# NVIDIA-Merlin/NVTabular

Measured on AMD Instinct MI355X. Metric: rows/sec + GB/s (Criteo Categorify+FillMissing+Normalize fit+transform, HBM-resident), higher is better.
Workload: dtype int32 keys -> int64 labels; fp64 moments/normalize; 1 GPU; synthetic Criteo-day0: 26 int32 categorical (Criteo-1TB cardinalities, Zipf) + 13 int32 continuous, nulls as Arrow bitmaps; Categorify + FillMissing + Normalize, fit + transform; rows_per_gpu=45000000, algorithmic_bytes_per_row=624, tie_break=value (count desc, value asc), artifacts=deferred (no parquet I/O inside the timed region)

## Files before the change

### nvtabular_amd/csrc/nvt_sort.hip

```cpp
#include <type_traits>

#include <cstdlib>
#include <vector>

#include "nvt_common.hpp"
#include "nvt_internal.hpp"
#include "nvt_prof.hpp"
#include "nvt_range.hpp"
#include "nvt_image.hpp"
#include "nvt_scan.hpp"

extern "C" int nvt_vocab_sort_tmp_bytes(int key_bytes, uint64_t n, uint64_t *bytes);

namespace nvt {

template <typename K>
__device__ __forceinline__ unsigned sort_digit(K key, int64_t cnt, int pass) {
  constexpr int KB = (int)sizeof(K);
  if (pass < KB) {
    using U = typename std::make_unsigned<K>::type;
    U u = (U)key ^ ((U)1 << (8 * KB - 1));
    return (unsigned)((u >> (8 * pass)) & 0xFF);
  }
  uint64_t inv = ~(uint64_t)cnt;
  return (unsigned)((inv >> (8 * (pass - KB))) & 0xFF);
}

constexpr int kSmallMax = 8192;
constexpr int kSmallBS = 1024;

template <typename K>
__device__ __forceinline__ bool vocab_before(int64_t ca, K ka, int64_t cb, K kb) {
  return ca > cb || (ca == cb && ka < kb);
}

template <typename K>
__global__ __launch_bounds__(kSmallBS) void sort_small_kernel(K *keys, int64_t *counts, unsigned n) {
  __shared__ K sk[kSmallMax];
  __shared__ int64_t sc[kSmallMax];
  unsigned m = 1;
  while (m < n) m <<= 1;
  for (unsigned i = threadIdx.x; i < m; i += kSmallBS) {
    if (i < n) {
      sk[i] = keys[i];
      sc[i] = counts[i];
    } else {
      sk[i] = std::numeric_limits<K>::max();
      sc[i] = INT64_MIN;
    }
  }
  __syncthreads();
  for (unsigned size = 2; size <= m; size <<= 1) {
    for (unsigned stride = size >> 1; stride > 0; stride >>= 1) {
      for (unsigned t = threadIdx.x; t < m / 2; t += kSmallBS) {
        unsigned lo = 2 * t - (t & (stride - 1));
        unsigned hi = lo + stride;
        bool up = (lo & size) == 0;
        K ka = sk[lo], kb = sk[hi];
        int64_t ca = sc[lo], cb = sc[hi];
        bool swap = up ? vocab_before<K>(cb, kb, ca, ka) : vocab_before<K>(ca, ka, cb, kb);
        if (swap) {
          sk[lo] = kb;
          sk[hi] = ka;
          sc[lo] = cb;
          sc[hi] = ca;
        }
      }
      __syncthreads();
    }
  }
  for (unsigned i = threadIdx.x; i < n; i += kSmallBS) {
    keys[i] = sk[i];
    counts[i] = sc[i];
  }
}

constexpr int kRows = 8;
constexpr int kTileSort = kBlock * kRows;

template <typename K>
__global__ __launch_bounds__(kBlock) void sort_pass_hist_kernel(const K *__restrict__ keys,
                                                                const int64_t *__restrict__ cnts,
                                                                uint64_t n,
                                                                unsigned long long *pass_hist) {
// ... 564 lines not shown
}

uint64_t sort_words_tmp_bytes(uint64_t n) { return os_tmp_bytes(n); }

static int sort_words_impl(uint64_t *data, const void *keys, int key_dtype, int64_t key_bias,
                           const uint8_t *fold, int rb, uint64_t n, int bit_lo, int bit_hi, void *tmp,
                           uint64_t **result, hipStream_t stream) {
  NVT_CHECK_ARG(n < (1ull << 30), "at most 2^30-1 words");
  const int npass = (bit_hi - bit_lo + 7) / 8;
  NVT_CHECK_ARG(npass >= 1 && npass <= kOsMaxPass, "bit range too wide");
  const uint64_t ntiles = (n + kS2Tile - 1) / kS2Tile;
  char *p = reinterpret_cast<char *>(tmp);
  uint64_t *bufs[2];
  bufs[0] = reinterpret_cast<uint64_t *>(p);
  p += n * 8;
  bufs[1] = reinterpret_cast<uint64_t *>(p);
  p += n * 8;
  unsigned *block_hist = reinterpret_cast<unsigned *>(p);
  p += (uint64_t)kOsHistBlocks * kOsMaxPass * 256 * 4;
  unsigned *base = reinterpret_cast<unsigned *>(p);
  p += kOsMaxPass * 256 * 4;
  unsigned *status = reinterpret_cast<unsigned *>(p);
  const uint64_t status_words = (uint64_t)npass * ntiles * 256;
  unsigned *tickets = status + status_words;
  NVT_CHECK_HIP(hipMemsetAsync(status, 0, (status_words + kOsMaxPass) * 4, stream));
  const unsigned hb = (unsigned)(ntiles < (uint64_t)kOsHistBlocks ? ntiles : kOsHistBlocks);
  const PackedKeyWord<int32_t> s32{reinterpret_cast<const int32_t *>(keys), fold, key_bias, rb};
  const PackedKeyWord<int64_t> s64{reinterpret_cast<const int64_t *>(keys), fold, key_bias, rb};
  if (!keys)
    os_hist_words_kernel<<<hb, kS2BS, 0, stream>>>(data, n, bit_lo, npass, block_hist);
  else if (key_dtype == NVT_I32)
    os_hist_pack_kernel<int32_t><<<hb, kS2BS, 0, stream>>>(s32, n, bit_lo, npass, block_hist);
  else
    os_hist_pack_kernel<int64_t><<<hb, kS2BS, 0, stream>>>(s64, n, bit_lo, npass, block_hist);
  NVT_CHECK_LAUNCH();
  os_base_kernel<<<npass, 256, 0, stream>>>(block_hist, (int)hb, base);
  NVT_CHECK_LAUNCH();
  const uint64_t *src = data;
  int flip = 0;
  for (int pass = 0; pass < npass; ++pass) {
    uint64_t *dst = bufs[flip];
    unsigned *st = status + (uint64_t)pass * ntiles * 256;
    if (pass == 0 && keys && key_dtype == NVT_I32)
      os_scatter_pack_kernel<int32_t><<<(unsigned)ntiles, kS2BS, 0, stream>>>(
          s32, n, bit_lo, base, st, tickets, dst);
    else if (pass == 0 && keys)
      os_scatter_pack_kernel<int64_t><<<(unsigned)ntiles, kS2BS, 0, stream>>>(
          s64, n, bit_lo, base, st, tickets, dst);
    else
      os_scatter_kernel<false, false><<<(unsigned)ntiles, kS2BS, 0, stream>>>(
          src, nullptr, nullptr, n, bit_lo + 8 * pass, base + pass * 256, st, tickets + pass, dst,
          nullptr, nullptr);
    NVT_CHECK_LAUNCH();
    src = dst;
    flip ^= 1;
  }
  *result = const_cast<uint64_t *>(src);
  return NVT_OK;
}

int sort_words_bits(uint64_t *data, uint64_t n, int bit_lo, int bit_hi, void *tmp, uint64_t **result,
                    hipStream_t stream) {
  *result = data;
  if (n <= 1 || bit_hi <= bit_lo) return NVT_OK;
  return sort_words_impl(data, nullptr, 0, 0, nullptr, 0, n, bit_lo, bit_hi, tmp, result, stream);
}

int sort_packed_keys(const void *keys, int key_dtype, int64_t key_bias, const uint8_t *fold, int rb,
                     uint64_t n, void *tmp, uint64_t **result, hipStream_t stream) {
  NVT_CHECK_ARG(keys && n >= 1 && rb >= 24 && rb <= 32, "keys / rows / row bits");
  return sort_words_impl(nullptr, keys, key_dtype, key_bias, fold, rb, n, rb, 64, tmp, result, stream);
}

constexpr int kSmallPackedMax = 16384;
struct SmallCol {
  int32_t *keys;
  int64_t *counts;
  unsigned n;
};
constexpr int kSmallBatch = 64;
struct SmallBatch {
  SmallCol c[kSmallBatch];
};
__global__ __launch_bounds__(kSmallBS) void sort_small_packed_many_kernel(SmallBatch b) {
  __shared__ uint64_t sv[kSmallPackedMax];
  const SmallCol col = b.c[blockIdx.x];
  const unsigned n = col.n;
  unsigned m = 1;
  while (m < n) m <<= 1;
  for (unsigned i = threadIdx.x; i < m; i += kSmallBS)
    sv[i] = i < n ? comp_make(col.keys[i], col.counts[i]) : ~0ull;
  __syncthreads();
  for (unsigned size = 2; size <= m; size <<= 1) {
    for (unsigned stride = size >> 1; stride > 0; stride >>= 1) {
      for (unsigned t = threadIdx.x; t < m / 2; t += kSmallBS) {
        const unsigned lo = 2 * t - (t & (stride - 1));
        const unsigned hi = lo + stride;
        const bool up = (lo & size) == 0;
        const uint64_t a = sv[lo], c = sv[hi];
        if (up ? (c < a) : (a < c)) {
          sv[lo] = c;
          sv[hi] = a;
        }
      }
      __syncthreads();
    }
  }
  for (unsigned i = threadIdx.x; i < n; i += kSmallBS) {
    const uint64_t v = sv[i];
    col.keys[i] = comp_key(v);
    col.counts[i] = comp_cnt(v);
  }
}

inline uint64_t sort2_tmp_bytes(uint64_t n) {
  const uint64_t ntiles = (n + kS2Tile - 1) / kS2Tile, hist_len = 256 * ntiles;
  return 2 * n * 8 + pad16(hist_len * 4) + scan_chunks(hist_len) * 8 + 64;
}

inline int vocab_sort_packed(int32_t *keys, int64_t *counts, uint64_t n, int64_t max_count,
                             void *tmp, hipStream_t stream) {
  const uint64_t ntiles = (n + kS2Tile - 1) / kS2Tile, hist_len = 256 * ntiles;
  char *p = reinterpret_cast<char *>(tmp);
  uint64_t *bufs[2];
  bufs[0] = reinterpret_cast<uint64_t *>(p);
  p += n * 8;
  bufs[1] = reinterpret_cast<uint64_t *>(p);
  p += n * 8;
  unsigned *tile_hist = reinterpret_cast<unsigned *>(p);
  p += pad16(hist_len * 4);
  unsigned long long *chunk_tot = reinterpret_cast<unsigned long long *>(p);
  int count_bytes = 0;
  for (uint64_t m = (uint64_t)max_count; m; m >>= 8) ++count_bytes;
  const int npass = 4 + count_bytes;
  const uint64_t *src = nullptr;
  int flip = 0;
  for (int pass = 0; pass < npass; ++pass) {
    const int shift = 8 * pass;
    const bool first = pass == 0, last = pass == npass - 1;
    if (first)
      sort2_hist_kernel<true><<<(unsigned)ntiles, kS2BS, 0, stream>>>(nullptr, keys, counts, n,
                                                                       shift, tile_hist, ntiles);
    else
      sort2_hist_kernel<false><<<(unsigned)ntiles, kS2BS, 0, stream>>>(src, nullptr, nullptr, n,
                                                                        shift, tile_hist, ntiles);
    NVT_CHECK_LAUNCH();
    const unsigned long long *cbase = nullptr;
    {
      int rc = exclusive_scan_u32_deferred(tile_hist, hist_len, chunk_tot, &cbase, stream);
      if (rc) return rc;
    }
    uint64_t *dst = bufs[flip];
    if (first)
      sort2_scatter_kernel<true, false><<<(unsigned)ntiles, kS2BS, 0, stream>>>(
          nullptr, keys, counts, n, shift, tile_hist, cbase, ntiles, dst, nullptr, nullptr);
    else if (last)
      sort2_scatter_kernel<false, true><<<(unsigned)ntiles, kS2BS, 0, stream>>>(
          src, nullptr, nullptr, n, shift, tile_hist, cbase, ntiles, nullptr, keys, counts);
    else
      sort2_scatter_kernel<false, false><<<(unsigned)ntiles, kS2BS, 0, stream>>>(
          src, nullptr, nullptr, n, shift, tile_hist, cbase, ntiles, dst, nullptr, nullptr);
    NVT_CHECK_LAUNCH();
    src = dst;
    flip ^= 1;
  }
  return NVT_OK;
}

template <typename K>
int vocab_sort(K *keys, int64_t *counts, uint64_t n, int64_t max_count, void *tmp,
               hipStream_t stream) {
  constexpr int NP = (int)sizeof(K) + 8;
  if (n <= 1) return NVT_OK;
  NVT_CHECK_ARG(n < (1ull << 32), "at most 2^32-1 vocabulary entries");
  if (n <= kSmallMax) {
    sort_small_kernel<K><<<1, kSmallBS, 0, stream>>>(keys, counts, (unsigned)n);
    NVT_CHECK_LAUNCH();
    return NVT_OK;
  }
  if constexpr (sizeof(K) == 4) {
    if (max_count > 0 && max_count < (1ll << 32) && n < (1ull << 30) && !ab_env("NVT_SORT_LEGACY"))
      return vocab_sort_onesweep(keys, counts, n, max_count, tmp, stream);
    if (max_count > 0 && max_count < (1ll << 32) && n < (1ull << 31))
      return vocab_sort_packed(keys, counts, n, max_count, tmp, stream);
  }
  const uint64_t ntiles = (n + kTileSort - 1) / kTileSort;
  char *p = reinterpret_cast<char *>(tmp);
  int64_t *counts2 = reinterpret_cast<int64_t *>(p);
  p += n * sizeof(int64_t);
  K *keys2 = reinterpret_cast<K *>(p);
  p += pad16(n * sizeof(K));
  unsigned *tile_hist = reinterpret_cast<unsigned *>(p);
  const uint64_t hist_len = 256 * ntiles;
  p += pad16(hist_len * sizeof(unsigned));
  const uint64_t nchunks = (hist_len + kScanChunk - 1) / kScanChunk;
  unsigned long long *chunk_tot = reinterpret_cast<unsigned long long *>(p);
  p += nchunks * sizeof(unsigned long long);
  unsigned long long *pass_hist = reinterpret_cast<unsigned long long *>(p);

  bool run_pass[NP];
  if (max_count > 0) {
    constexpr int KB = (int)sizeof(K);
    int count_bytes = 0;
    for (uint64_t m = (uint64_t)max_count; m; m >>= 8) ++count_bytes;
    for (int p = 0; p < NP; ++p) run_pass[p] = p < KB || (p - KB) < count_bytes;
  } else {
    NVT_CHECK_HIP(hipMemsetAsync(pass_hist, 0, NP * 256 * sizeof(unsigned long long), stream));
    sort_pass_hist_kernel<K><<<stream_grid(n, kBlock * 8, 4), kBlock, 0, stream>>>(keys, counts, n,
                                                                                     pass_hist);
    NVT_CHECK_LAUNCH();
    unsigned long long host_hist[NP * 256];
    NVT_CHECK_HIP(hipMemcpyAsync(host_hist, pass_hist, sizeof(host_hist), hipMemcpyDeviceToHost,
                                 stream));
    NVT_CHECK_HIP(hipStreamSynchronize(stream));
    for (int p = 0; p < NP; ++p) {
      run_pass[p] = true;
      for (int d = 0; d < 256; ++d)
        if (host_hist[p * 256 + d] == n) run_pass[p] = false;
    }
  }

  K *src_k = keys, *dst_k = keys2;
  int64_t *src_c = counts, *dst_c = counts2;
  for (int pass = 0; pass < NP; ++pass) {
    if (!run_pass[pass]) continue;
    sort_tile_hist_kernel<K><<<(unsigned)ntiles, kBlock, 0, stream>>>(src_k, src_c, n, pass,
                                                                      tile_hist, ntiles);
    NVT_CHECK_LAUNCH();
    {
      int rc = exclusive_scan_u32(tile_hist, hist_len, chunk_tot, stream);
      if (rc) return rc;
    }
    sort_scatter_kernel<K><<<(unsigned)ntiles, kBlock, 0, stream>>>(src_k, src_c, n, pass,
                                                                    tile_hist, ntiles, dst_k, dst_c);
    NVT_CHECK_LAUNCH();
    K *tk = src_k;
    src_k = dst_k;
    dst_k = tk;
    int64_t *tc = src_c;
    src_c = dst_c;
    dst_c = tc;
  }
  if (src_k != keys) {
    NVT_CHECK_HIP(hipMemcpyAsync(keys, src_k, n * sizeof(K), hipMemcpyDeviceToDevice, stream));
    NVT_CHECK_HIP(
        hipMemcpyAsync(counts, src_c, n * sizeof(int64_t), hipMemcpyDeviceToDevice, stream));
  }
  return NVT_OK;
}

int vocab_sort_any(int key_bytes, void *keys, int64_t *counts, uint64_t n, int64_t max_count,
                   void *tmp, hipStream_t s) {
  NVT_PROF("vocab_sort", 0, s);
  if (key_bytes == 4) return vocab_sort<int32_t>((int32_t *)keys, counts, n, max_count, tmp, s);
  return vocab_sort<int64_t>((int64_t *)keys, counts, n, max_count, tmp, s);
}

bool vocab_sort_small_eligible(int key_bytes, uint64_t n, int64_t max_count) {
  return key_bytes == 4 && n >= 2 && n <= (uint64_t)kSmallPackedMax && max_count > 0 &&
         max_count < (1ll << 32);
}

int vocab_sort_small_batch(const SmallSortDesc *cols, int ncols, hipStream_t s) {
  for (int c0 = 0; c0 < ncols; c0 += kSmallBatch) {
    const int nc = ncols - c0 < kSmallBatch ? ncols - c0 : kSmallBatch;
    SmallBatch b;
    memset(&b, 0, sizeof(b));
    for (int i = 0; i < nc; ++i) {
      b.c[i].keys = cols[c0 + i].keys;
      b.c[i].counts = cols[c0 + i].counts;
      b.c[i].n = cols[c0 + i].n;
    }
    NVT_PROF("vocab_sort_small", 0, s);
    sort_small_packed_many_kernel<<<nc, kSmallBS, 0, s>>>(b);
    NVT_CHECK_LAUNCH();
  }
  return NVT_OK;
}

__device__ __forceinline__ unsigned cls_digit(uint64_t comp) {
  const uint32_t cnt = ~(uint32_t)(comp >> 32);
  return 255u - (cnt < 255u ? cnt : 255u);
}

__device__ __forceinline__ void cls_scatter_body(
    const int32_t *__restrict__ keys, const int64_t *__restrict__ cnts, uint64_t n,
    const unsigned *__restrict__ cls_hist, unsigned *status, unsigned *ticket, int32_t *out_keys,
    int64_t *out_cnts, unsigned long long *table, uint64_t mask, int64_t first_label,
    int64_t *sentinel_label, int32_t *label_of, int32_t *big_src = nullptr) {
  constexpr int NW = kS2BS / kWave;
  __shared__ unsigned wcnt[NW][256];
  __shared__ unsigned goff[256];
  __shared__ unsigned wtot[NW], btot[NW];
  __shared__ unsigned s_tile;
  __shared__ uint64_t stage[kS2Tile];
  const unsigned w = threadIdx.x / kWave, l = lane_id();
  if (threadIdx.x == 0) s_tile = atomicAdd(ticket, 1u);
#pragma unroll
  for (int q = 0; q < NW; ++q) wcnt[q][threadIdx.x] = 0;
  unsigned cbase;
  {
    const unsigned v = cls_hist[255 - threadIdx.x];
    unsigned inc = v;
#pragma unroll
    for (int off = 1; off < 64; off <<= 1) {
      unsigned o = __shfl_up(inc, off, 64);
      if (l >= (unsigned)off) inc += o;
    }
    if (l == 63) btot[w] = inc;
    __syncthreads();
    unsigned wb = 0;
    for (unsigned q = 0; q < w; ++q) wb += btot[q];
    cbase = wb + inc - v;
  }
  const unsigned tile = s_tile;
  uint64_t c[kS2Rows];
  unsigned short local[kS2Rows];
#pragma unroll
  for (int r = 0; r < kS2Rows; ++r) {
    const uint64_t i = s2_elem(tile, w, r, l);
    c[r] = ~0ull;
    if (i < n) c[r] = comp_make(keys[i], cnts[i]);
  }
  const uint64_t tile_base = (uint64_t)tile * kS2Tile;
#pragma unroll
  for (int r = 0; r < kS2Rows; ++r) {
    const bool act = s2_elem(tile, w, r, l) < n;
    const unsigned d = cls_digit(c[r]);
    const unsigned long long peers = match_digit(d, act);
    const unsigned rank = __popcll(peers & ((1ull << l) - 1ull));
    const unsigned before = act ? wcnt[w][d] : 0;
    __builtin_amdgcn_wave_barrier();
    if (act && rank == 0) wcnt[w][d] = before + (unsigned)__popcll(peers);
    __builtin_amdgcn_wave_barrier();
    local[r] = (unsigned short)(before + rank);
  }
  __syncthreads();
  {
    const unsigned d = threadIdx.x;
    unsigned t[NW], tot = 0;
#pragma unroll
    for (int q = 0; q < NW; ++q) {
      t[q] = wcnt[q][d];
      tot += t[q];
    }
    unsigned *my = status + (uint64_t)tile * 256 + d;
    __hip_atomic_store(my, (tile == 0 ? kOsPrefix : kOsAgg) | tot, __ATOMIC_RELAXED,
                       __HIP_MEMORY_SCOPE_AGENT);
    unsigned inc = tot;
#pragma unroll
    for (int off = 1; off < 64; off <<= 1) {
      unsigned o = __shfl_up(inc, off, 64);
      if (l >= (unsigned)off) inc += o;
    }
    if (l == 63) wtot[w] = inc;
    __syncthreads();
    unsigned wbase = 0;
    for (unsigned q = 0; q < w; ++q) wbase += wtot[q];
    const unsigned dstart = wbase + inc - tot;
    unsigned run = dstart;
#pragma unroll
    for (int q = 0; q < NW; ++q) {
      wcnt[q][d] = run;
      run += t[q];
    }
    unsigned excl = 0;
    if (tile > 0) {
      unsigned tb = tile - 1;
      while (true) {
        const unsigned v = __hip_atomic_load(status + (uint64_t)tb * 256 + d, __ATOMIC_RELAXED,
                                             __HIP_MEMORY_SCOPE_AGENT);
        const unsigned f = v >> 30;
        if (f == 0) {
          __builtin_amdgcn_s_sleep(1);
          continue;
        }
        excl += v & kOsMask;
        if (f == 2) break;
        --tb;
      }
      __hip_atomic_store(my, kOsPrefix | (excl + tot), __ATOMIC_RELAXED, __HIP_MEMORY_SCOPE_AGENT);
    }
    goff[d] = cbase + excl - dstart;
  }
  __syncthreads();
#pragma unroll
  for (int r = 0; r < kS2Rows; ++r) {
    const uint64_t i = s2_elem(tile, w, r, l);
    if (i < n) {
      const unsigned d = cls_digit(c[r]);
      const unsigned sidx = wcnt[w][d] + local[r];
      stage[sidx] = c[r];
      if (label_of != nullptr) label_of[i] = d != 0 ? (int32_t)(first_label + goff[d] + sidx) : -1;
      if (big_src != nullptr && d == 0) big_src[goff[0] + sidx] = (int32_t)i;
    }
  }
  __syncthreads();
  const unsigned tile_n = (unsigned)(n - tile_base < (uint64_t)kS2Tile ? n - tile_base : kS2Tile);
#pragma unroll 4
  for (int j = 0; j < kS2Rows; ++j) {
    const unsigned idx = j * kS2BS + threadIdx.x;
    if (idx < tile_n) {
      const uint64_t v = stage[idx];
      const unsigned d = cls_digit(v);
      if (big_src != nullptr && d != 0) continue;
      const unsigned dst = goff[d] + idx;
      const int32_t key = comp_key(v);
      out_keys[dst] = key;
      out_cnts[dst] = comp_cnt(v);
      if (key == INT32_MIN && d != 0 && sentinel_label != nullptr) {
        *sentinel_label = first_label + (int64_t)dst;
      } else if (table != nullptr && d != 0) {
        const int64_t label = first_label + (int64_t)dst;
        {
          const unsigned long long want = ((unsigned long long)(uint32_t)label << 32) | (uint32_t)key;
          uint64_t slot = (uint64_t)slot_hash(key) & mask;
          while (atomicCAS(&table[slot], kEncEmptySlot, want) != kEncEmptySlot) slot = (slot + 1) & mask;
        }
      }
    }
  }
}

__global__ __launch_bounds__(kS2BS) void cls_scatter_kernel(
    const int32_t *__restrict__ keys, const int64_t *__restrict__ cnts, uint64_t n,
    const unsigned *__restrict__ cls_hist, unsigned *status, unsigned *ticket, int32_t *out_keys,
    int64_t *out_cnts, unsigned long long *table, uint64_t mask, int64_t first_label,
    int64_t *sentinel_label, int32_t *label_of) {
  cls_scatter_body(keys, cnts, n, cls_hist, status, ticket, out_keys, out_cnts, table, mask,
                   first_label, sentinel_label, label_of);
}

constexpr int kOrdBatch = 16;
struct OrdJob {
  const int32_t *keys;
  const int64_t *cnts;
  const unsigned *cls_hist;
  unsigned *status, *ticket;
  int32_t *out_keys;
  int64_t *out_cnts;
  int32_t *label_of;
  unsigned long long *table;
  int64_t *sentinel_label;
  int32_t *aux;
  unsigned long long *fb_status;
  unsigned long long n, capacity, nslots, flat_slots, first_label, status_words, fb_words;
};
struct OrdBatch {
  OrdJob j[kOrdBatch];
  unsigned tile_start[kOrdBatch + 1];
  unsigned flat_start[kOrdBatch + 1];
  int njobs;
};
__device__ __forceinline__ int ord_job_of(const unsigned *start, int n, unsigned b) {
  int c = 0;
  while (c + 1 < n && b >= start[c + 1]) ++c;
  return c;
}

__global__ __launch_bounds__(kBlock) void ord_prep_kernel(OrdBatch b) {
  const OrdJob &j = b.j[blockIdx.y];
  const uint64_t stride = (uint64_t)gridDim.x * kBlock;
  const uint64_t t0 = (uint64_t)blockIdx.x * kBlock + threadIdx.x;
  for (uint64_t i = t0; i < j.status_words; i += stride) j.status[i] = 0;
  for (uint64_t i = t0; i < j.fb_words; i += stride) j.fb_status[i] = 0;
  if (j.flat_slots) {
    for (uint64_t i = t0; i < j.capacity; i += stride) j.table[i] = kEncEmptySlot;
  }
  if (t0 == 0) *j.sentinel_label = -1;
}

__global__ __launch_bounds__(kS2BS) void cls_scatter_many_kernel(OrdBatch b) {
  const int ji = ord_job_of(b.tile_start, b.njobs, blockIdx.x);
  const OrdJob &j = b.j[ji];
  cls_scatter_body(j.keys, j.cnts, j.n, j.cls_hist, j.status, j.ticket, j.out_keys, j.out_cnts,
                   nullptr, 0, (int64_t)j.first_label, j.sentinel_label, j.label_of);
}

__global__ __launch_bounds__(kBlock) void range_patch_kernel(unsigned long long *table,
                                                             uint64_t nslots,
                                                             const int32_t *__restrict__ label_of) {
  const uint64_t stride = (uint64_t)gridDim.x * kBlock * 2;
  for (uint64_t s0 = ((uint64_t)blockIdx.x * kBlock + threadIdx.x) * 2; s0 < nslots; s0 += stride) {
    ulonglong2 e = *reinterpret_cast<ulonglong2 *>(table + s0);
    bool dirty = false;
    if ((int32_t)(uint32_t)e.x != INT32_MIN) {
      e.x = ((unsigned long long)(uint32_t)label_of[(uint32_t)(e.x >> 32)] << 32) | (uint32_t)e.x;
      dirty = true;
    }
    if ((int32_t)(uint32_t)e.y != INT32_MIN) {
      e.y = ((unsigned long long)(uint32_t)label_of[(uint32_t)(e.y >> 32)] << 32) | (uint32_t)e.y;
      dirty = true;
    }
    if (dirty) *reinterpret_cast<ulonglong2 *>(table + s0) = e;
  }
}

__global__ __launch_bounds__(kBlock) void range_fix_prefix_kernel(
    unsigned long long *table, const int32_t *__restrict__ aux, const int32_t *__restrict__ vocab,
    uint64_t n_big, int64_t first_label, int64_t *sentinel_label, uint64_t table_slots) {
  const RangeMap map = load_map(aux);
  const uint64_t stride = (uint64_t)gridDim.x * kBlock;
  for (uint64_t j = (uint64_t)blockIdx.x * kBlock + threadIdx.x; j < n_big; j += stride) {
    const int32_t key = vocab[j];
    const int64_t label = first_label + (int64_t)j;
    if (key == INT32_MIN) {
      *sentinel_label = label;
      continue;
    }
    uint64_t s = map.table_slot(key);
    if (map.flat) {
      s = flat_find_from(table, table_slots, s, key, table[s]);
      if (s != ~0ull) table[s] = ((unsigned long long)(uint32_t)label << 32) | (uint32_t)key;
      continue;
    }
    while (true) {
      const unsigned long long e = table[s];
      if ((int32_t)(uint32_t)e == key) {
        table[s] = ((unsigned long long)(uint32_t)label << 32) | (uint32_t)key;
        break;
      }
      if ((int32_t)(uint32_t)e == INT32_MIN) break;
      ++s;
    }
  }
}

__global__ __launch_bounds__(kBlock) void range_patch_many_kernel(OrdBatch b) {
  const OrdJob &j = b.j[blockIdx.y];
  if (j.flat_slots || j.nslots == 0) return;
  unsigned long long *table = j.table;
  const int32_t *__restrict__ label_of = j.label_of;
  const uint64_t nslots = j.nslots;
  const uint64_t stride = (uint64_t)gridDim.x * kBlock * 2;
  for (uint64_t s0 = ((uint64_t)blockIdx.x * kBlock + threadIdx.x) * 2; s0 < nslots; s0 += stride) {
    ulonglong2 e = *reinterpret_cast<ulonglong2 *>(table + s0);
    bool dirty = false;
    if ((int32_t)(uint32_t)e.x != INT32_MIN) {
      e.x = ((unsigned long long)(uint32_t)label_of[(uint32_t)(e.x >> 32)] << 32) | (uint32_t)e.x;
      dirty = true;
    }
    if ((int32_t)(uint32_t)e.y != INT32_MIN) {
      e.y = ((unsigned long long)(uint32_t)label_of[(uint32_t)(e.y >> 32)] << 32) | (uint32_t)e.y;
      dirty = true;
    }
    if (dirty) *reinterpret_cast<ulonglong2 *>(table + s0) = e;
  }
}

struct FixJob {
  unsigned long long *table;
  const int32_t *aux, *vocab;
  int64_t *sentinel_label;
  unsigned long long n_big, first_label, table_slots;
};
struct FixBatch {
  FixJob j[kOrdBatch];
};
__global__ __launch_bounds__(kBlock) void range_fix_prefix_many_kernel(FixBatch b) {
  const FixJob &f = b.j[blockIdx.y];
  const RangeMap map = load_map(f.aux);
  const uint64_t stride = (uint64_t)gridDim.x * kBlock;
  for (uint64_t j = (uint64_t)blockIdx.x * kBlock + threadIdx.x; j < f.n_big; j += stride) {
    const int32_t key = f.vocab[j];
    const int64_t label = (int64_t)f.first_label + (int64_t)j;
    if (key == INT32_MIN) {
      *f.sentinel_label = label;
      continue;
    }
    uint64_t s = map.table_slot(key);
    if (map.flat) {
      s = flat_find_from(f.table, f.table_slots, s, key, f.table[s]);
      if (s != ~0ull) f.table[s] = ((unsigned long long)(uint32_t)label << 32) | (uint32_t)key;
      continue;
    }
    while (true) {
      const unsigned long long e = f.table[s];
      if ((int32_t)(uint32_t)e == key) {
        f.table[s] = ((unsigned long long)(uint32_t)label << 32) | (uint32_t)key;
        break;
      }
      if ((int32_t)(uint32_t)e == INT32_MIN) break;
      ++s;
    }
  }
}

__global__ __launch_bounds__(kBlock) void class_hist_kernel(const int64_t *__restrict__ cnts,
                                                            uint64_t n, unsigned *hist) {
  __shared__ unsigned h[256];
  h[threadIdx.x] = 0;
  __syncthreads();
  const uint64_t stride = (uint64_t)gridDim.x * kBlock;
  unsigned ones = 0;
  for (uint64_t i = (uint64_t)blockIdx.x * kBlock + threadIdx.x; i < n; i += stride) {
    const int64_t c = cnts[i];
    if (c == 1)
      ++ones;
    else
      atomicAdd(&h[c < 255 ? (c < 0 ? 0 : (unsigned)c) : 255u], 1u);
  }
#pragma unroll
  for (int off = 32; off > 0; off >>= 1) ones += __shfl_down(ones, off, 64);
  if (lane_id() == 0 && ones) atomicAdd(&h[1], ones);
  __syncthreads();
  if (h[threadIdx.x]) atomicAdd(&hist[threadIdx.x], h[threadIdx.x]);
}

__device__ __forceinline__ void flat_params_body(const int32_t *__restrict__ keys, uint64_t n,
                                                 uint64_t slots, int32_t *aux) {
  const uint64_t first = (n > 1 && keys[0] == INT32_MIN) ? 1 : 0;
  const uint64_t lo = ukey(keys[first]), hi = ukey(keys[n - 1]);
  const uint64_t span = hi - lo, F = slots;
  uint32_t mul;
  int sh;
  range_map_params(span, F, &mul, &sh);
  aux[NVT_RANGE_AUX_LO] = (int32_t)(uint32_t)lo;
  aux[NVT_RANGE_AUX_LO + 1] = (int32_t)(uint32_t)span;
  aux[NVT_RANGE_AUX_LO + 2] = (int32_t)mul;
  aux[NVT_RANGE_AUX_LO + 3] = 0;
  aux[NVT_RANGE_AUX_LO + 4] = sh;
  aux[NVT_RANGE_AUX_LO + 5] = 1;
  aux[NVT_RANGE_AUX_LO + 6] = keys[0] == INT32_MIN ? 1 : 0;
  aux[NVT_FLAT_AUX_MAXDISP] = 0;
}
__global__ void flat_params_kernel(const int32_t *__restrict__ keys, uint64_t n, uint64_t slots,
                                   int32_t *aux) {
  flat_params_body(keys, n, slots, aux);
}
// ... 351 lines not shown
__global__ __launch_bounds__(kBlock) void label_scatter_kernel(
    const int32_t *__restrict__ keys, const int64_t *__restrict__ cnts, const int32_t *__restrict__ labels,
    uint64_t n, int64_t first_label, int32_t *__restrict__ out_keys, int64_t *__restrict__ out_cnts,
    int32_t *__restrict__ abs_label, int64_t *sentinel_label) {
  const uint64_t stride = (uint64_t)gridDim.x * kBlock;
  for (uint64_t i = (uint64_t)blockIdx.x * kBlock + threadIdx.x; i < n; i += stride) {
    const int32_t k = keys[i];
    const uint32_t l = (uint32_t)labels[i];
    out_keys[l] = k;
    out_cnts[l] = cnts[i];
    abs_label[i] = (int32_t)(first_label + (int64_t)l);
    if (k == INT32_MIN && sentinel_label != nullptr) *sentinel_label = first_label + (int64_t)l;
  }
}

int vocab_from_labels(const int32_t *src_keys, const int64_t *src_cnts, const int32_t *labels, uint64_t n,
                      int32_t *out_keys, int64_t *out_cnts, void *tmp, int64_t first_label, void *table,
                      uint64_t capacity, int64_t *sentinel_label, const int32_t *range_aux,
                      uint64_t flat_slots, hipStream_t s) {
  if (n == 0) return NVT_OK;
  NVT_CHECK_ARG(n < (1ull << 30), "at most 2^30-1 vocabulary entries");
  const uint64_t ntiles = (n + kS2Tile - 1) / kS2Tile;
  int32_t *abs_label = reinterpret_cast<int32_t *>(reinterpret_cast<char *>(tmp) + pad16(ntiles * 256 * 4 + 64));
  unsigned long long *fb_status =
      reinterpret_cast<unsigned long long *>(reinterpret_cast<char *>(abs_label) + pad16(n * 4));
  const bool flat = table != nullptr && range_aux != nullptr && flat_slots > 0;
  if (table != nullptr) {
    if (flat) {
      NVT_CHECK_ARG(flat_slots >= 64 && flat_slots < (1ull << 32), "flat table: 64 .. 2^32-1 slots");
      NVT_CHECK_ARG(capacity >= flat_slots + n + 64, "flat table: slots + n + 64");
    }
    int rc = encode_clear_any(4, table, capacity, sentinel_label, s);
    if (rc) return rc;
  }
  NVT_PROF("vocab_order", 0, s);
  label_scatter_kernel<<<stream_grid(n, kBlock, 8), kBlock, 0, s>>>(src_keys, src_cnts, labels, n, first_label,
                                                                    out_keys, out_cnts, abs_label,
                                                                    table != nullptr ? sentinel_label : nullptr);
  NVT_CHECK_LAUNCH();
  if (flat) {
    int32_t *aux = const_cast<int32_t *>(range_aux);
    flat_params_kernel<<<1, 1, 0, s>>>(src_keys, n, flat_slots, aux);
    NVT_CHECK_LAUNCH();
    NVT_CHECK_HIP(hipMemsetAsync(fb_status, 0, ntiles * 8 + 64, s));
    flat_build_kernel<<<(unsigned)ntiles, kS2BS, 0, s>>>(src_keys, abs_label, n, aux, fb_status,
                                                        reinterpret_cast<unsigned *>(fb_status + ntiles),
                                                        (unsigned long long *)table, capacity);
    NVT_CHECK_LAUNCH();
  } else if (table != nullptr) {
    int rc = encode_insert_any(4, out_keys, n, first_label, table, capacity, sentinel_label, s);
    if (rc) return rc;
  }
  return NVT_OK;
}

uint64_t vocab_order_tmp_bytes(uint64_t n, uint64_t n_big) {
  const uint64_t ntiles = (n + kS2Tile - 1) / kS2Tile;
  uint64_t sort_bytes = 0;
  if (n_big > 1) (void)nvt_vocab_sort_tmp_bytes(4, n_big, &sort_bytes);
  return pad16(ntiles * 256 * 4 + 64) + pad16(sort_bytes) + pad16(n * 4) + pad16(ntiles * 8 + 64) + 64;
}

int vocab_order_from_sorted(const int32_t *src_keys, const int64_t *src_cnts, uint64_t n,
                            const unsigned *cls_hist, uint64_t n_big, int64_t max_count,
                            int32_t *out_keys, int64_t *out_cnts, void *tmp, int64_t first_label,
                            void *table, uint64_t capacity, int64_t *sentinel_label,
                            const int32_t *range_aux, int range_nb_log2, hipStream_t s,
                            bool *tail_deferred, uint64_t flat_slots) {
  if (tail_deferred) *tail_deferred = false;
  if (n == 0) return NVT_OK;
  NVT_CHECK_ARG(n < (1ull << 30), "at most 2^30-1 vocabulary entries");
  NVT_CHECK_ARG(n_big <= n, "n_big > n");
  const uint64_t ntiles = (n + kS2Tile - 1) / kS2Tile;
  unsigned *status = reinterpret_cast<unsigned *>(tmp);
  unsigned *ticket = status + ntiles * 256;
  uint64_t sort_bytes = 0;
  if (n_big > 1) (void)nvt_vocab_sort_tmp_bytes(4, n_big, &sort_bytes);
  char *sort_tmp = reinterpret_cast<char *>(tmp) + pad16(ntiles * 256 * 4 + 64);
  int32_t *label_of = reinterpret_cast<int32_t *>(sort_tmp + pad16(sort_bytes));
  unsigned long long *fb_status =
      reinterpret_cast<unsigned long long *>(reinterpret_cast<char *>(label_of) + pad16(n * 4));
  const bool flat = table != nullptr && range_aux != nullptr && flat_slots > 0;
  const bool ranged = table != nullptr && range_aux != nullptr;
  if (flat) {
    NVT_CHECK_ARG(flat_slots >= 64 && flat_slots < (1ull << 32), "flat table: 64 .. 2^32-1 slots");
    NVT_CHECK_ARG(capacity >= flat_slots + n + 64, "flat table: slots + n + 64");
    int rc = encode_clear_any(4, table, capacity, sentinel_label, s);
    if (rc) return rc;
  } else if (table && !ranged) {
    int rc = encode_clear_any(4, table, capacity, sentinel_label, s);
    if (rc) return rc;
  } else if (ranged) {
    NVT_CHECK_HIP(hipMemsetAsync(sentinel_label, 0xFF, 8, s));
  }
  {
    NVT_PROF("vocab_order", 0, s);
    NVT_CHECK_HIP(hipMemsetAsync(status, 0, ntiles * 256 * 4 + 64, s));
    cls_scatter_kernel<<<(unsigned)ntiles, kS2BS, 0, s>>>(
        src_keys, src_cnts, n, cls_hist, status, ticket, out_keys, out_cnts,
        ranged ? nullptr : (unsigned long long *)table, capacity - 1, first_label, sentinel_label,
        ranged ? label_of : nullptr);
    NVT_CHECK_LAUNCH();
    if (flat) {
      int32_t *aux = const_cast<int32_t *>(range_aux);
      flat_params_kernel<<<1, 1, 0, s>>>(src_keys, n, flat_slots, aux);
      NVT_CHECK_LAUNCH();
      NVT_CHECK_HIP(hipMemsetAsync(fb_status, 0, ntiles * 8 + 64, s));
      flat_build_kernel<<<(unsigned)ntiles, kS2BS, 0, s>>>(
          src_keys, label_of, n, aux, fb_status, reinterpret_cast<unsigned *>(fb_status + ntiles),
          (unsigned long long *)table, capacity);
      NVT_CHECK_LAUNCH();
    } else if (ranged) {
      const uint64_t nslots = ((uint64_t)1 << range_nb_log2) * kRpRegion + kRpGuard;
      range_patch_kernel<<<stream_grid(nslots / 2, kBlock, 8), kBlock, 0, s>>>(
          (unsigned long long *)table, nslots, label_of);
      NVT_CHECK_LAUNCH();
    }
  }
  if (tail_deferred && vocab_sort_small_eligible(4, n_big, max_count)) {
    *tail_deferred = true;
    return NVT_OK;
  }
  if (n_big > 1) {
    int rc = vocab_sort_any(4, out_keys, out_cnts, n_big, max_count, sort_tmp, s);
    if (rc) return rc;
  }
  if (table && n_big > 0) {
    if (ranged) {
      NVT_PROF("encode_build", 0, s);
      range_fix_prefix_kernel<<<stream_grid(n_big, kBlock), kBlock, 0, s>>>(
          (unsigned long long *)table, range_aux, out_keys, n_big, first_label, sentinel_label,
          capacity);
      NVT_CHECK_LAUNCH();
    } else {
      int rc = encode_insert_any(4, out_keys, n_big, first_label, table, capacity, sentinel_label, s);
      if (rc) return rc;
    }
  }
  return NVT_OK;
}

int vocab_order_sorted_batch(const OrderSortedJob *jobs, int njobs, hipStream_t s) {
  for (int j0 = 0; j0 < njobs; j0 += kOrdBatch) {
    const int nj = njobs - j0 < kOrdBatch ? njobs - j0 : kOrdBatch;
    OrdBatch b;
    memset(&b, 0, sizeof(b));
    std::vector<OrderTail> tails;
    bool any_flat = false, any_ranged = false;
    for (int i = 0; i < nj; ++i) {
      const OrderSortedJob &q = jobs[j0 + i];
      NVT_CHECK_ARG(q.n > 0 && q.n < (1ull << 30), "1 .. 2^30-1 vocabulary entries");
      NVT_CHECK_ARG(q.n_big <= q.n, "n_big > n");
      NVT_CHECK_ARG(q.table && q.range_aux && q.tmp && q.sentinel_label, "range table jobs only");
      const uint64_t ntiles = (q.n + kS2Tile - 1) / kS2Tile;
      unsigned *status = reinterpret_cast<unsigned *>(q.tmp);
      uint64_t sort_bytes = 0;
      if (q.n_big > 1) (void)nvt_vocab_sort_tmp_bytes(4, q.n_big, &sort_bytes);
      char *sort_tmp = reinterpret_cast<char *>(q.tmp) + pad16(ntiles * 256 * 4 + 64);
      int32_t *label_of = reinterpret_cast<int32_t *>(sort_tmp + pad16(sort_bytes));
      OrdJob &o = b.j[i];
      o.keys = q.src_keys;
      o.cnts = q.src_cnts;
      o.cls_hist = q.cls_hist;
      o.status = status;
      o.ticket = status + ntiles * 256;
      o.out_keys = q.out_keys;
      o.out_cnts = q.out_cnts;
      o.label_of = label_of;
      o.table = reinterpret_cast<unsigned long long *>(q.table);
      o.sentinel_label = q.sentinel_label;
      o.aux = const_cast<int32_t *>(q.range_aux);
      o.fb_status = reinterpret_cast<unsigned long long *>(reinterpret_cast<char *>(label_of) + pad16(q.n * 4));
      o.n = q.n;
      o.capacity = q.capacity;
      o.flat_slots = q.flat_slots;
      o.nslots = q.flat_slots ? 0 : ((uint64_t)1 << q.range_nb_log2) * kRpRegion + kRpGuard;
      o.first_label = (unsigned long long)q.first_label;
      o.status_words = ntiles * 256 + 16;
      o.fb_words = q.flat_slots ? ntiles + 8 : 0;
      if (q.flat_slots) {
        NVT_CHECK_ARG(q.flat_slots >= 64 && q.flat_slots < (1ull << 32), "flat table: 64 .. 2^32-1 slots");
        NVT_CHECK_ARG(q.capacity >= q.flat_slots + q.n + 64, "flat table: slots + n + 64");
        any_flat = true;
      } else {
        any_ranged = true;
      }
      b.tile_start[i + 1] = b.tile_start[i] + (unsigned)ntiles;
      b.flat_start[i + 1] = b.flat_start[i] + (q.flat_slots ? (unsigned)ntiles : 0u);
    }
    b.njobs = nj;
    {
      NVT_PROF("vocab_order", 0, s);
      ord_prep_kernel<<<dim3(any_flat ? 2048 : 64, nj), kBlock, 0, s>>>(b);
      NVT_CHECK_LAUNCH();
      cls_scatter_many_kernel<<<b.tile_start[nj], kS2BS, 0, s>>>(b);
      NVT_CHECK_LAUNCH();
      if (any_flat) {
        flat_params_many_kernel<<<nj, 1, 0, s>>>(b);
        NVT_CHECK_LAUNCH();
        flat_build_many_kernel<<<b.flat_start[nj], kS2BS, 0, s>>>(b);
        NVT_CHECK_LAUNCH();
      }
      if (any_ranged) {
        range_patch_many_kernel<<<dim3(1024, nj), kBlock, 0, s>>>(b);
        NVT_CHECK_LAUNCH();
      }
    }
    for (int i = 0; i < nj; ++i) {
      const OrderSortedJob &q = jobs[j0 + i];
      if (q.n_big == 0) continue;
      if (vocab_sort_small_eligible(4, q.n_big, q.max_count)) {
        tails.push_back({q.out_keys, q.out_cnts, q.n_big, q.first_label, q.table, q.capacity,
                         q.sentinel_label, q.range_aux});
        continue;
      }
      if (q.n_big > 1) {
        const uint64_t ntiles = (q.n + kS2Tile - 1) / kS2Tile;
        char *sort_tmp = reinterpret_cast<char *>(q.tmp) + pad16(ntiles * 256 * 4 + 64);
        int rc = vocab_sort_any(4, q.out_keys, q.out_cnts, q.n_big, q.max_count, sort_tmp, s);
        if (rc) return rc;
      }
      NVT_PROF("encode_build", 0, s);
      range_fix_prefix_kernel<<<stream_grid(q.n_big, kBlock), kBlock, 0, s>>>(
          (unsigned long long *)q.table, q.range_aux, q.out_keys, q.n_big, q.first_label,
          q.sentinel_label, q.capacity);
      NVT_CHECK_LAUNCH();
    }
    if (!tails.empty()) {
      int rc = vocab_order_tail_batch(tails.data(), (int)tails.size(), s);
      if (rc) return rc;
    }
  }
  return NVT_OK;
}

int vocab_order_tail_batch(const OrderTail *t, int nt, hipStream_t s) {
  if (nt == 0) return NVT_OK;
  std::vector<SmallSortDesc> d(nt);
  for (int i = 0; i < nt; ++i) {
    d[i].keys = t[i].keys;
    d[i].counts = t[i].counts;
    d[i].n = (unsigned)t[i].n_big;
  }
  int rc = vocab_sort_small_batch(d.data(), nt, s);
  if (rc) return rc;
  NVT_PROF("encode_build", 0, s);
  for (int i0 = 0; i0 < nt;) {
    FixBatch fb;
    memset(&fb, 0, sizeof(fb));
    int nf = 0;
    uint64_t longest = 0;
    for (; i0 < nt && nf < kOrdBatch; ++i0) {
      if (!t[i0].table || !t[i0].range_aux) continue;
      fb.j[nf++] = {(unsigned long long *)t[i0].table, t[i0].range_aux, t[i0].keys,
                    t[i0].sentinel_label, t[i0].n_big, (unsigned long long)t[i0].first_label,
                    t[i0].capacity};
      longest = t[i0].n_big > longest ? t[i0].n_big : longest;
    }
    if (nf) {
      range_fix_prefix_many_kernel<<<dim3(stream_grid(longest, kBlock), nf), kBlock, 0, s>>>(fb);
      NVT_CHECK_LAUNCH();
    }
  }
  for (int i = 0; i < nt; ++i) {
    if (!t[i].table) continue;
    if (t[i].range_aux) {
      continue;
    } else {
      rc = encode_insert_any(4, t[i].keys, t[i].n_big, t[i].first_label, t[i].table, t[i].capacity,
                             t[i].sentinel_label, s);
      if (rc) return rc;
    }
  }
  return NVT_OK;
}

}

using namespace nvt;

extern "C" {

int nvt_vocab_sort_tmp_bytes(int key_bytes, uint64_t n, uint64_t *bytes) {
  NVT_CHECK_ARG(bytes && (key_bytes == 4 || key_bytes == 8), "key_bytes must be 4 or 8");
  const uint64_t ntiles = (n + kTileSort - 1) / kTileSort;
  const uint64_t hist_len = 256 * ntiles;
  const uint64_t nchunks = (hist_len + kScanChunk - 1) / kScanChunk;
// ... 318 lines not shown
```

Measured before the change: 5.017 billion rows/s.

## Fuse range-table label patch into class scatter; register bitonic small sort

For ranged (non-flat) tables, the class-scatter kernel now probes the range hash table directly and writes final labels during scatter. This removes the separate range_patch pass, which swept every table slot and gathered through label_of. The small vocabulary sort now does its bitonic stages in registers with wave shuffles and uses shared memory only for strides wider than a wave's span. Its block size is derived from the column size. The tradeoff is extra register pressure and probing work inside the scatter kernel.

```diff
diff --git a/nvtabular_amd/csrc/nvt_sort.hip b/nvtabular_amd/csrc/nvt_sort.hip
--- a/nvtabular_amd/csrc/nvt_sort.hip
+++ b/nvtabular_amd/csrc/nvt_sort.hip
@@ -1,5 +1,6 @@
 #include <type_traits>
 
+#include <algorithm>
 #include <cstdlib>
 #include <vector>
 
@@ -730,18 +731,58 @@
 struct SmallBatch {
   SmallCol c[kSmallBatch];
 };
-__global__ __launch_bounds__(kSmallBS) void sort_small_packed_many_kernel(SmallBatch b) {
-  __shared__ uint64_t sv[kSmallPackedMax];
-  const SmallCol col = b.c[blockIdx.x];
-  const unsigned n = col.n;
-  unsigned m = 1;
-  while (m < n) m <<= 1;
-  for (unsigned i = threadIdx.x; i < m; i += kSmallBS)
-    sv[i] = i < n ? comp_make(col.keys[i], col.counts[i]) : ~0ull;
-  __syncthreads();
-  for (unsigned size = 2; size <= m; size <<= 1) {
-    for (unsigned stride = size >> 1; stride > 0; stride >>= 1) {
-      for (unsigned t = threadIdx.x; t < m / 2; t += kSmallBS) {
+template <int E>
+__device__ __forceinline__ void small_wave_merge(uint64_t (&v)[E], unsigned base, unsigned l,
+                                                 unsigned size) {
+#pragma unroll
+  for (int js = E / 2; js > 0; js >>= 1) {
+    if ((unsigned)js * 64 >= size) continue;
+#pragma unroll
+    for (int e = 0; e < E; ++e) {
+      if (e & js) continue;
+      const bool up = ((base + e * 64 + l) & size) == 0;
+      const uint64_t a = v[e], c = v[e | js];
+      const bool sw = up ? (c < a) : (a < c);
+      v[e] = sw ? c : a;
+      v[e | js] = sw ? a : c;
+    }
+  }
+#pragma unroll
+  for (int st = 32; st > 0; st >>= 1) {
+    if ((unsigned)st >= size) continue;
+    const bool lower = (l & st) == 0;
+#pragma unroll
+    for (int e = 0; e < E; ++e) {
+      const bool up = ((base + e * 64 + l) & size) == 0;
+      const uint64_t mine = v[e];
+      const uint64_t o = (uint64_t)__shfl_xor((unsigned long long)mine, st, 64);
+      v[e] = (lower == up) ? (o < mine ? o : mine) : (o > mine ? o : mine);
+    }
+  }
+}
+
+template <int E>
+__device__ __forceinline__ void small_sort_body(const SmallCol &col, uint64_t *sv, unsigned m) {
+  constexpr unsigned W = 64 * E;
+  const unsigned n = col.n, l = lane_id();
+  const unsigned base = (threadIdx.x / kWave) * W;
+  const bool live = base < m;
+  uint64_t v[E];
+#pragma unroll
+  for (int e = 0; e < E; ++e) {
+    const unsigned i = base + e * 64 + l;
+    v[e] = (live && i < n) ? comp_make(col.keys[i], col.counts[i]) : ~0ull;
+  }
+  if (live)
+    for (unsigned size = 2; size <= W; size <<= 1) small_wave_merge<E>(v, base, l, size);
+  for (unsigned size = 2 * W; size <= m; size <<= 1) {
+    if (live) {
+#pragma unroll
+      for (int e = 0; e < E; ++e) sv[base + e * 64 + l] = v[e];
+    }
+    __syncthreads();
+    for (unsigned stride = size >> 1; stride >= W; stride >>= 1) {
+      for (unsigned t = threadIdx.x; t < m / 2; t += blockDim.x) {
         const unsigned lo = 2 * t - (t & (stride - 1));
         const unsigned hi = lo + stride;
         const bool up = (lo & size) == 0;
@@ -753,12 +794,41 @@
       }
       __syncthreads();
     }
-  }
-  for (unsigned i = threadIdx.x; i < n; i += kSmallBS) {
-    const uint64_t v = sv[i];
-    col.keys[i] = comp_key(v);
-    col.counts[i] = comp_cnt(v);
-  }
+    if (live) {
+#pragma unroll
+      for (int e = 0; e < E; ++e) v[e] = sv[base + e * 64 + l];
+      small_wave_merge<E>(v, base, l, size);
+    }
+  }
+  if (live) {
+#pragma unroll
+    for (int e = 0; e < E; ++e) {
+      const unsigned i = base + e * 64 + l;
+      if (i < n) {
+        col.keys[i] = comp_key(v[e]);
+        col.counts[i] = comp_cnt(v[e]);
+      }
+    }
+  }
+}
+
+constexpr unsigned kSmallWide = 8192;
+inline unsigned small_sort_waves(unsigned n) {
+  unsigned m = 1;
+  while (m < n) m <<= 1;
+  if (m > kSmallWide) return m / (64 * 16);
+  return m > 64 * 8 ? m / (64 * 8) : 1u;
+}
+
+__global__ __launch_bounds__(kSmallBS) void sort_small_packed_many_kernel(SmallBatch b) {
+  __shared__ uint64_t sv[kSmallPackedMax];
+  const SmallCol col = b.c[blockIdx.x];
+  unsigned m = 1;
+  while (m < col.n) m <<= 1;
+  if (m > kSmallWide)
+    small_sort_body<16>(col, sv, m);
+  else
+    small_sort_body<8>(col, sv, m < 64 * 8 ? 64 * 8 : m);
 }
 
 inline uint64_t sort2_tmp_bytes(uint64_t n) {
@@ -914,13 +984,16 @@
     const int nc = ncols - c0 < kSmallBatch ? ncols - c0 : kSmallBatch;
     SmallBatch b;
     memset(&b, 0, sizeof(b));
+    unsigned waves = 1;
     for (int i = 0; i < nc; ++i) {
       b.c[i].keys = cols[c0 + i].keys;
       b.c[i].counts = cols[c0 + i].counts;
       b.c[i].n = cols[c0 + i].n;
+      NVT_CHECK_ARG(cols[c0 + i].n <= (unsigned)kSmallPackedMax, "small sort: at most 16384 entries");
+      waves = std::max(waves, small_sort_waves(cols[c0 + i].n));
     }
     NVT_PROF("vocab_sort_small", 0, s);
-    sort_small_packed_many_kernel<<<nc, kSmallBS, 0, s>>>(b);
+    sort_small_packed_many_kernel<<<nc, waves * kWave, 0, s>>>(b);
     NVT_CHECK_LAUNCH();
   }
   return NVT_OK;
@@ -935,17 +1008,24 @@
     const int32_t *__restrict__ keys, const int64_t *__restrict__ cnts, uint64_t n,
     const unsigned *__restrict__ cls_hist, unsigned *status, unsigned *ticket, int32_t *out_keys,
     int64_t *out_cnts, unsigned long long *table, uint64_t mask, int64_t first_label,
-    int64_t *sentinel_label, int32_t *label_of, int32_t *big_src = nullptr) {
+    int64_t *sentinel_label, int32_t *label_of, int32_t *big_src = nullptr,
+    unsigned long long *rtable = nullptr, const int32_t *raux = nullptr, uint64_t rslots = 0) {
   constexpr int NW = kS2BS / kWave;
   __shared__ unsigned wcnt[NW][256];
   __shared__ unsigned goff[256];
   __shared__ unsigned wtot[NW], btot[NW];
   __shared__ unsigned s_tile;
   __shared__ uint64_t stage[kS2Tile];
+  __shared__ uint32_t s_pw[kRpPwWords];
   const unsigned w = threadIdx.x / kWave, l = lane_id();
   if (threadIdx.x == 0) s_tile = atomicAdd(ticket, 1u);
 #pragma unroll
   for (int q = 0; q < NW; ++q) wcnt[q][threadIdx.x] = 0;
+  RangeMap rmap = {};
+  if (rtable != nullptr) {
+    rmap = load_map(raux);
+    stage_pieces(rmap, s_pw, threadIdx.x, kS2BS);
+  }
   unsigned cbase;
   {
     const unsigned v = cls_hist[255 - threadIdx.x];
@@ -1041,6 +1121,49 @@
       stage[sidx] = c[r];
       if (label_of != nullptr) label_of[i] = d != 0 ? (int32_t)(first_label + goff[d] + sidx) : -1;
       if (big_src != nullptr && d == 0) big_src[goff[0] + sidx] = (int32_t)i;
+    }
+  }
+  if (rtable != nullptr) {
+    constexpr int G = 8;
+#pragma unroll
+    for (int r0 = 0; r0 < kS2Rows; r0 += G) {
+      uint64_t sl[G];
+      unsigned long long want[G];
+      bool pend[G];
+#pragma unroll
+      for (int q = 0; q < G; ++q) {
+        const int r = r0 + q;
+        const unsigned d = cls_digit(c[r]);
+        const int32_t key = comp_key(c[r]);
+        pend[q] = s2_elem(tile, w, r, l) < n && d != 0 && key != INT32_MIN;
+        sl[q] = 0;
+        want[q] = 0;
+        if (pend[q]) {
+          const int64_t label = first_label + (int64_t)(goff[d] + wcnt[w][d] + local[r]);
+          want[q] = ((unsigned long long)(uint32_t)label << 32) | (uint32_t)key;
+          sl[q] = rmap.table_slot(key);
+        }
+      }
+      bool any = true;
+      while (any) {
+        unsigned long long e[G];
+#pragma unroll
+        for (int q = 0; q < G; ++q) e[q] = (pend[q] && sl[q] < rslots) ? rtable[sl[q]] : kEncEmptySlot;
+        any = false;
+#pragma unroll
+        for (int q = 0; q < G; ++q) {
+          if (!pend[q]) continue;
+          if ((uint32_t)e[q] == (uint32_t)want[q]) {
+            rtable[sl[q]] = want[q];
+            pend[q] = false;
+          } else if ((int32_t)(uint32_t)e[q] == INT32_MIN) {
+            pend[q] = false;
+          } else {
+            ++sl[q];
+            any = true;
+          }
+        }
+      }
     }
   }
   __syncthreads();
@@ -1074,9 +1197,10 @@
     const int32_t *__restrict__ keys, const int64_t *__restrict__ cnts, uint64_t n,
     const unsigned *__restrict__ cls_hist, unsigned *status, unsigned *ticket, int32_t *out_keys,
     int64_t *out_cnts, unsigned long long *table, uint64_t mask, int64_t first_label,
-    int64_t *sentinel_label, int32_t *label_of) {
+    int64_t *sentinel_label, int32_t *label_of, unsigned long long *rtable, const int32_t *raux,
+    uint64_t rslots) {
   cls_scatter_body(keys, cnts, n, cls_hist, status, ticket, out_keys, out_cnts, table, mask,
-                   first_label, sentinel_label, label_of);
+                   first_label, sentinel_label, label_of, nullptr, rtable, raux, rslots);
 }
 
 constexpr int kOrdBatch = 16;
@@ -1121,27 +1245,11 @@
 __global__ __launch_bounds__(kS2BS) void cls_scatter_many_kernel(OrdBatch b) {
   const int ji = ord_job_of(b.tile_start, b.njobs, blockIdx.x);
   const OrdJob &j = b.j[ji];
+  const bool dumped = j.flat_slots == 0 && j.nslots != 0;
   cls_scatter_body(j.keys, j.cnts, j.n, j.cls_hist, j.status, j.ticket, j.out_keys, j.out_cnts,
-                   nullptr, 0, (int64_t)j.first_label, j.sentinel_label, j.label_of);
-}
-
-__global__ __launch_bounds__(kBlock) void range_patch_kernel(unsigned long long *table,
-                                                             uint64_t nslots,
-                                                             const int32_t *__restrict__ label_of) {
-  const uint64_t stride = (uint64_t)gridDim.x * kBlock * 2;
-  for (uint64_t s0 = ((uint64_t)blockIdx.x * kBlock + threadIdx.x) * 2; s0 < nslots; s0 += stride) {
-    ulonglong2 e = *reinterpret_cast<ulonglong2 *>(table + s0);
-    bool dirty = false;
-    if ((int32_t)(uint32_t)e.x != INT32_MIN) {
-      e.x = ((unsigned long long)(uint32_t)label_of[(uint32_t)(e.x >> 32)] << 32) | (uint32_t)e.x;
-      dirty = true;
-    }
-    if ((int32_t)(uint32_t)e.y != INT32_MIN) {
-      e.y = ((unsigned long long)(uint32_t)label_of[(uint32_t)(e.y >> 32)] << 32) | (uint32_t)e.y;
-      dirty = true;
-    }
-    if (dirty) *reinterpret_cast<ulonglong2 *>(table + s0) = e;
-  }
+                   nullptr, 0, (int64_t)j.first_label, j.sentinel_label,
+                   dumped ? nullptr : j.label_of, nullptr, dumped ? j.table : nullptr, j.aux,
+                   j.nslots);
 }
 
 __global__ __launch_bounds__(kBlock) void range_fix_prefix_kernel(
@@ -1171,28 +1279,6 @@
       if ((int32_t)(uint32_t)e == INT32_MIN) break;
       ++s;
     }
-  }
-}
-
-__global__ __launch_bounds__(kBlock) void range_patch_many_kernel(OrdBatch b) {
-  const OrdJob &j = b.j[blockIdx.y];
-  if (j.flat_slots || j.nslots == 0) return;
-  unsigned long long *table = j.table;
-  const int32_t *__restrict__ label_of = j.label_of;
-  const uint64_t nslots = j.nslots;
-  const uint64_t stride = (uint64_t)gridDim.x * kBlock * 2;
-  for (uint64_t s0 = ((uint64_t)blockIdx.x * kBlock + threadIdx.x) * 2; s0 < nslots; s0 += stride) {
-    ulonglong2 e = *reinterpret_cast<ulonglong2 *>(table + s0);
-    bool dirty = false;
-    if ((int32_t)(uint32_t)e.x != INT32_MIN) {
-      e.x = ((unsigned long long)(uint32_t)label_of[(uint32_t)(e.x >> 32)] << 32) | (uint32_t)e.x;
-      dirty = true;
-    }
-    if ((int32_t)(uint32_t)e.y != INT32_MIN) {
-      e.y = ((unsigned long long)(uint32_t)label_of[(uint32_t)(e.y >> 32)] << 32) | (uint32_t)e.y;
-      dirty = true;
-    }
-    if (dirty) *reinterpret_cast<ulonglong2 *>(table + s0) = e;
   }
 }
 
@@ -1710,6 +1796,8 @@
       reinterpret_cast<unsigned long long *>(reinterpret_cast<char *>(label_of) + pad16(n * 4));
   const bool flat = table != nullptr && range_aux != nullptr && flat_slots > 0;
   const bool ranged = table != nullptr && range_aux != nullptr;
+  const bool dumped = ranged && !flat;
+  const uint64_t dumped_slots = dumped ? ((uint64_t)1 << range_nb_log2) * kRpRegion + kRpGuard : 0;
   if (flat) {
     NVT_CHECK_ARG(flat_slots >= 64 && flat_slots < (1ull << 32), "flat table: 64 .. 2^32-1 slots");
     NVT_CHECK_ARG(capacity >= flat_slots + n + 64, "flat table: slots + n + 64");
@@ -1727,7 +1815,8 @@
     cls_scatter_kernel<<<(unsigned)ntiles, kS2BS, 0, s>>>(
         src_keys, src_cnts, n, cls_hist, status, ticket, out_keys, out_cnts,
         ranged ? nullptr : (unsigned long long *)table, capacity - 1, first_label, sentinel_label,
-        ranged ? label_of : nullptr);
+        flat ? label_of : nullptr, dumped ? (unsigned long long *)table : nullptr, range_aux,
+        dumped_slots);
     NVT_CHECK_LAUNCH();
     if (flat) {
       int32_t *aux = const_cast<int32_t *>(range_aux);
@@ -1738,11 +1827,6 @@
           src_keys, label_of, n, aux, fb_status, reinterpret_cast<unsigned *>(fb_status + ntiles),
           (unsigned long long *)table, capacity);
       NVT_CHECK_LAUNCH();
-    } else if (ranged) {
-      const uint64_t nslots = ((uint64_t)1 << range_nb_log2) * kRpRegion + kRpGuard;
-      range_patch_kernel<<<stream_grid(nslots / 2, kBlock, 8), kBlock, 0, s>>>(
-          (unsigned long long *)table, nslots, label_of);
-      NVT_CHECK_LAUNCH();
     }
   }
   if (tail_deferred && vocab_sort_small_eligible(4, n_big, max_count)) {
@@ -1774,7 +1858,7 @@
     OrdBatch b;
     memset(&b, 0, sizeof(b));
     std::vector<OrderTail> tails;
-    bool any_flat = false, any_ranged = false;
+    bool any_flat = false;
     for (int i = 0; i < nj; ++i) {
       const OrderSortedJob &q = jobs[j0 + i];
       NVT_CHECK_ARG(q.n > 0 && q.n < (1ull << 30), "1 .. 2^30-1 vocabulary entries");
@@ -1810,8 +1894,6 @@
         NVT_CHECK_ARG(q.flat_slots >= 64 && q.flat_slots < (1ull << 32), "flat table: 64 .. 2^32-1 slots");
         NVT_CHECK_ARG(q.capacity >= q.flat_slots + q.n + 64, "flat table: slots + n + 64");
         any_flat = true;
-      } else {
-        any_ranged = true;
       }
       b.tile_start[i + 1] = b.tile_start[i] + (unsigned)ntiles;
       b.flat_start[i + 1] = b.flat_start[i] + (q.flat_slots ? (unsigned)ntiles : 0u);
@@ -1827,10 +1909,6 @@
         flat_params_many_kernel<<<nj, 1, 0, s>>>(b);
         NVT_CHECK_LAUNCH();
         flat_build_many_kernel<<<b.flat_start[nj], kS2BS, 0, s>>>(b);
-        NVT_CHECK_LAUNCH();
-      }
-      if (any_ranged) {
-        range_patch_many_kernel<<<dim3(1024, nj), kBlock, 0, s>>>(b);
         NVT_CHECK_LAUNCH();
       }
     }
```

Measured after the change: 5.038 billion rows/s, median of 3. About the same (+0.4%).
